# michel-aractingi/soloRL

Hardware: AMD Instinct MI355X
Metric: env-steps/s (whole node) Solo12 walk, 4096 envs/GPU (higher is better)
Workload: dtype f32

## Files before the change

### solorl_amd/csrc/dynamics.hpp

```cpp
#pragma once
#include <utility>

#include "../../include/solorl.h"
#include "../../include/solorl_model_data.h"
#include "spatial.hpp"

namespace solo {

constexpr int MAX_CONTACTS = 8;
constexpr int MAX_LIMITS = 4;
constexpr int LIM_SLOT_ROWS = 2;
constexpr int MAX_ROWS = LIM_SLOT_ROWS + 3 * MAX_CONTACTS;
SD int extra_limits(int nlt) { return nlt > LIM_SLOT_ROWS ? nlt - LIM_SLOT_ROWS : 0; }
SD int contact_cap(int nlt) { return MAX_CONTACTS - extra_limits(nlt); }
constexpr int ROW_CORE = 20;
constexpr int NPRIM = 24;
constexpr double LIMIT_WINDOW = 0.0;
constexpr double DISC_EPS2 = 1e-12;
constexpr double DISC_RIM = 0.1;

#if defined(SOLO_WAVE_TIMING) && !defined(SOLO_HOST_SHIM)
constexpr int SOLO_WT_WAVES = 65536, SOLO_WT_FIELDS = 30;
__device__ unsigned long long solo_wave_times[SOLO_WT_WAVES][SOLO_WT_FIELDS];
__shared__ unsigned long long solo_pt_acc[12];
// ... 1841 lines not shown
    T nz = cw * z + ax * yq - ay * x + az * ww;
    T nq = cw * ww - ax * x - ay * yq - az * z;
    T inv = rsqrt_fast(nx * nx + ny * ny + nz * nz + nq * nq);
    C.ps.qx = nx * inv; C.ps.qy = ny * inv; C.ps.qz = nz * inv; C.ps.qw = nq * inv;
  }
}

template <typename T, int ROBOT, typename LDS> struct TeamCtx {
  using type = CtxLds<T, ROBOT, TeamRows<T, LDS>::off_ctx>;
  static constexpr size_t bytes = TeamRows<T, LDS>::off_ctx + 4 * sizeof(SubCtx<T, ROBOT>);
};

template <typename T, int ROBOT, typename LDS, typename CH>
SNI_SCALAR void duo_helper_rates(CH ch, const PhysParams<T> pp, const LDS lds, int t, bool valid) {
  if (valid) phase_legrates_team<T, ROBOT, LDS, CH>(ch, pp, lds, t);
  WG_SYNC();
}

template <typename T, int ROBOT>
SNI_SCALAR void duo_join_rows() {
  WG_SYNC();
}

template <typename T, int ROBOT, typename LDS, typename CH>
SNI_SCALAR void duo_integrate_joints(CH ch, const PhysParams<T> pp, const LDS lds, int t, bool valid) {
  using RB = Robot<ROBOT>;
  using TRW = TeamRows<T, LDS>;
  constexpr int NJ = RB::NJ, LN = LDS::LANES;
  if (!valid) return;
  SubCtx<T, ROBOT>& C = ch.get();
  const T dt = pp.dt;
  const int mask = C.mask;
  const int nlt = C.nlim_total;
  const T* hdr = lds.hdr();
  const SV<T> w{{hdr[2 * LN], hdr[3 * LN], hdr[4 * LN]}, {hdr[5 * LN], hdr[6 * LN], hdr[7 * LN]}};
  const int tj = t < RB::NQ ? t : 0;
  const int L = tj / NJ, k = tj - L * NJ;
  const T qds = C.qds[tj], yk = lds.y()[(L * 3 + k) * LN], qj = C.ps.q[tj];
  const SV<T> Gk = C.LR[L].G[k];
  const T* lam = TRW::lam(lds.lane);
  const int npos0 = TRW::NPOS0 + extra_limits(nlt);
  T lv[(NPRIM + 15) / 16];
#pragma unroll
  for (int i = 0; i < (NPRIM + 15) / 16; i++) {
    const int p = t + 16 * i;
    const int pp_ = p < NPRIM ? p : 0;
    lv[i] = lam[(npos0 + __builtin_popcount(mask & ((1 << pp_) - 1))) * 4];
    lv[i] = (p < NPRIM && ((mask >> pp_) & 1)) ? lv[i] : T(0);
  }
  const T nvj = clampv(qds + yk - dot(Gk, w), pp.vmax);
#pragma unroll
  for (int i = 0; i < (NPRIM + 15) / 16; i++) { const int p = t + 16 * i; if (p < NPRIM) C.lamp[p] = lv[i]; }
  if (t < RB::NQ) { C.ps.qd[t] = nvj; C.ps.q[t] = qj + dt * nvj; }
}

template <typename T, int ROBOT, typename LDS, typename CH>
SNI_SCALAR void duo_integrate_base(CH ch, const PhysParams<T> pp, const LDS lds, bool lead, bool r0) {
  constexpr int LN = LDS::LANES;
  if (!lead) return;
  SubCtx<T, ROBOT>& C = ch.get();
  const T dt = pp.dt;
  const T* hdr = lds.hdr();
  const SV<T> w{{hdr[2 * LN], hdr[3 * LN], hdr[4 * LN]}, {hdr[5 * LN], hdr[6 * LN], hdr[7 * LN]}};
  const SV<T> ub = C.ub;
  const V3<T> pos = C.ps.pos;
  const T x = C.ps.qx, yq = C.ps.qy, z = C.ps.qz, ww = C.ps.qw;
  const V3<T> nw = mk(clampv(ub.a.x + w.a.x, pp.vmax), clampv(ub.a.y + w.a.y, pp.vmax), clampv(ub.a.z + w.a.z, pp.vmax));
  const V3<T> nv = mk(clampv(ub.l.x + w.l.x, pp.vmax), clampv(ub.l.y + w.l.y, pp.vmax), clampv(ub.l.z + w.l.z, pp.vmax));
  C.ps.w = nw; C.ps.v = nv;
  C.ps.pos = fma3(nv, dt, pos);
  T wn2 = dot(nw, nw), wn = sqrt_fast(wn2), sc, s_, cw;
  sincos_t(T(0.5) * wn * dt, s_, cw);
  if (wn < T(1e-3)) sc = T(0.5) * dt - dt * dt * dt * T(1.0 / 48.0) * wn2; else sc = s_ * rcp_fast(wn);
  T ax = nw.x * sc, ay = nw.y * sc, az = nw.z * sc;
  T nx = cw * x + ax * ww + ay * z - az * yq;
  T ny = cw * yq - ax * z + ay * ww + az * x;
  T nz = cw * z + ax * yq - ay * x + az * ww;
  T nq = cw * ww - ax * x - ay * yq - az * z;
  T inv = rsqrt_fast(nx * nx + ny * ny + nz * nz + nq * nq);
  C.ps.qx = nx * inv; C.ps.qy = ny * inv; C.ps.qz = nz * inv; C.ps.qw = nq * inv;
  if (r0) C.R0 = quat_to_mat(C.ps.qx, C.ps.qy, C.ps.qz, C.ps.qw);
}

template <typename T, int ROBOT, typename LDS>
SD void substep_team_helper(const PhysParams<T> pp, const LDS& lds, int t, bool lead, bool valid, bool r0_next) {
  using CH = typename TeamCtx<T, ROBOT, LDS>::type;
  const CH ch{lds.lane};
  WG_SYNC();
  if (pp.urdf_inertia()) phase_front_team<T, ROBOT, LDS, CH, true, true>(ch, pp, lds, t, valid, lead);
  else phase_front_team<T, ROBOT, LDS, CH, false, true>(ch, pp, lds, t, valid, lead);
  WG_SYNC();
#if defined(SOLO_WAVE_TIMING)
  __builtin_amdgcn_s_waitcnt(0);
  const long long wt_h0_ = clock64();
#endif
  if (valid) team_sum_base<T, ROBOT, CH>(ch, t);
  if (lead) phase_base_lead<T, ROBOT, LDS, CH>(ch, pp, nullptr, 0u, lds);
  else if (!valid && t == 0) {
    lds.hdr()[0] = T(0); lds.hdr()[LDS::LANES] = T(0);
  }
#if defined(SOLO_WAVE_TIMING)
  __builtin_amdgcn_s_waitcnt(0);
  if (threadIdx.x == 64) solo_pt_acc[4] += (unsigned long long)(clock64() - wt_h0_);
#endif
  duo_helper_rates<T, ROBOT, LDS, CH>(ch, pp, lds, t, valid);
  duo_join_rows<T, ROBOT>();
#if defined(SOLO_WAVE_TIMING)
  __builtin_amdgcn_s_waitcnt(0);
  const long long wt_h1_ = clock64();
#endif
  duo_integrate_base<T, ROBOT, LDS, CH>(ch, pp, lds, lead, r0_next);
#if defined(SOLO_WAVE_TIMING)
  __builtin_amdgcn_s_waitcnt(0);
  if (threadIdx.x == 64) solo_pt_acc[11] += (unsigned long long)(clock64() - wt_h1_);
#endif
}

template <typename T, int ROBOT, typename LDS, bool DUO = false>
SD int substep_team(const PhysParams<T> pp, T* lam_prev, unsigned nstride, const LDS& lds, int t, bool lead, bool valid) {
  constexpr int LN = LDS::LANES;
  using TRW = TeamRows<T, LDS>;
  using CH = typename TeamCtx<T, ROBOT, LDS>::type;
  const CH ch{lds.lane};
  SOLO_PT_DECL();
  SOLO_PT_BEGIN();
  if (valid && t < Robot<ROBOT>::NQ) {
    SubCtx<T, ROBOT>& C = ch.get();
    T sn, cs;
    sincos_t(C.ps.q[t], sn, cs);
    C.sn[t] = sn; C.cs[t] = cs;
  }
  SOLO_PT(0);
  const bool ui = pp.urdf_inertia();
  if constexpr (DUO) WG_SYNC();
  else if (ui) phase_front_team<T, ROBOT, LDS, CH, true>(ch, pp, lds, t, valid, lead);
  else phase_front_team<T, ROBOT, LDS, CH, false>(ch, pp, lds, t, valid, lead);
  SOLO_PT(1);
#if SOLO_LEG_QUAD
  if constexpr (DUO) {
    if (ui) phase_leg_rt<T, ROBOT, LDS, CH, true, true>(ch, pp, lam_prev, nstride, lds, t >> 2, t & 3);
    else phase_leg_rt<T, ROBOT, LDS, CH, false, true>(ch, pp, lam_prev, nstride, lds, t >> 2, t & 3);
  } else if (valid) {
    if (ui) phase_leg_rt<T, ROBOT, LDS, CH, true>(ch, pp, lam_prev, nstride, lds, t >> 2, t & 3);
    else phase_leg_rt<T, ROBOT, LDS, CH, false>(ch, pp, lam_prev, nstride, lds, t >> 2, t & 3);
  }
#else
  static_assert(!DUO, "the helper wavefront's barrier B is in the quad leg phase");
  if (valid && t < 4) {
    if (ui) phase_leg_rt<T, ROBOT, LDS, CH, true>(ch, pp, lam_prev, nstride, lds, t, 0);
    else phase_leg_rt<T, ROBOT, LDS, CH, false>(ch, pp, lam_prev, nstride, lds, t, 0);
  }
#endif
  SOLO_PT(2);
  if constexpr (DUO) {
    duo_join_rows<T, ROBOT>();
    SOLO_PT(3);
  } else {
    if (valid) team_sum_base<T, ROBOT, CH>(ch, t);
    SOLO_PT(3);
    if (lead) phase_base_lead<T, ROBOT, LDS, CH>(ch, pp, lam_prev, nstride, lds);
    else if (!valid && t == 0) {
      lds.hdr()[0] = T(0); lds.hdr()[LN] = T(0);
    }
    SOLO_PT(4);
    if (valid) phase_legrates_team<T, ROBOT, LDS, CH>(ch, pp, lds, t);
    SOLO_PT(5);
  }
  phase_finish_team<T, ROBOT, LDS>(pp, lds, t);
  SOLO_PT(6);
  phase_pgs_team<T, ROBOT, LDS>(pp.iterations, pp.warm != T(0), pp.resid_thr >= T(0), pp.pgs_pipe(), pp.cone(), lds, t);
  SOLO_PT(7);
  if constexpr (DUO) {
    duo_join_rows<T, ROBOT>();
    SOLO_PT(10);
    duo_integrate_joints<T, ROBOT, LDS, CH>(ch, pp, lds, t, valid);
  } else phase_integrate_team<T, ROBOT, LDS, CH>(ch, pp, lam_prev, nstride, lds, t, valid, lead);
  SOLO_PT(8);
  return lead ? (ch.get().mask | strip_feet_bits(ch.get().smask)) : 0;
}
#endif

template <typename T, int ROBOT, typename LDS>
SD int substep(SubCtx<T, ROBOT>& C, const PhysParams<T> pp, T* lam_prev, unsigned nstride, const LDS& lds) {
  using CH = CtxPriv<T, ROBOT>;
  const CH ch{&C};
  if (pp.urdf_inertia()) {
    phase_detect<T, ROBOT, CH, true>(ch, pp);
    phase_leg<T, ROBOT, 0, LDS, CH, true>(ch, pp, lam_prev, nstride, lds);
// ... 19 lines not shown
```

### solorl_amd/csrc/solorl_hip.hip

```cpp
#include <hip/hip_runtime.h>

#include <cmath>
#include <cstddef>
#include <cstdio>
#include <cstdlib>
#include <cstring>
#include <utility>
#include <string>
#include <vector>

#include "../../include/solorl.h"
#include "dynamics.hpp"

using namespace solo;

#ifndef SOLO_TU_PART
#define SOLO_TU_PART -1
#endif
extern "C" __attribute__((visibility("hidden"))) int solorl_fail_(int code, const char* msg);

namespace {

#if SOLO_TU_PART == -1 || SOLO_TU_PART == 4
thread_local std::string g_err;
// ... 335 lines not shown
      for (int j = 0; j < NQ; j++) C.tau[j] = tau[j] * sc;
      E.mask = substep<T, ROBOT>(C, pp, sf + SX(L.lam, e, L.NF), 4u, lds);
    }
    E.ps = C.ps;
  }
  if (P.task == SOLORL_TASK_POINTGOAL && mode == MODE_STEP) pointgoal_progress(E, P, P.id0 + (long long)env);
  if (mode == MODE_SETTLE) { store_env(E, sf, si, L, (idx_t)N, e); return; }
  E.timestep += 1;
  const int done = reward_termination_outputs<T, NQ>(E, P, asq, out, env, N);

  if (done) reset_from_snapshot<T, ROBOT>(E, sf, L, (idx_t)N, e, env, snf, sni, M, P);
  write_obs<T, ROBOT>(E, sf, L, (idx_t)N, e, env, P.task, out.obs);
  store_env(E, sf, si, L, (idx_t)N, e);
}

#ifdef SOLO_WAVE_TIMING
#define WT_STAMP(i) do { wts_[i] = clock64(); } while (0)
#else
#define WT_STAMP(i) do {} while (0)
#endif

template <typename T> SD T team_sum16(T x) {
  if constexpr (sizeof(T) == 4) {
    x += __int_as_float(__builtin_amdgcn_mov_dpp(__float_as_int(x), 0xB1, 0xF, 0xF, true));
    x += __int_as_float(__builtin_amdgcn_mov_dpp(__float_as_int(x), 0x4E, 0xF, 0xF, true));
    x += __int_as_float(__builtin_amdgcn_mov_dpp(__float_as_int(x), 0x141, 0xF, 0xF, true));
    x += __int_as_float(__builtin_amdgcn_mov_dpp(__float_as_int(x), 0x140, 0xF, 0xF, true));
  } else {
    x += __shfl_xor(x, 1, 16); x += __shfl_xor(x, 2, 16); x += __shfl_xor(x, 4, 16); x += __shfl_xor(x, 8, 16);
  }
  return x;
}
enum { ER_GOAL = 0, ER_POT = 2, ER_PROG = 3, ER_GOALS = 4, ER_EGOALS = 5, ER_DR = 6, ER_XYPREV = 11, ER_TMY = 13, NER = 14 };
enum { IR_TIMESTEP = 0, IR_MASK = 1, IR_RNG = 2, IR_SNAP = 3, IR_DONE = 4 };
template <typename T, int ROBOT> SD void env_from_lds(Env<T, Robot<ROBOT>::NQ>& E, const SubCtx<T, ROBOT>& C) {
  E.ps = C.ps;
  E.goal[0] = C.erec[ER_GOAL]; E.goal[1] = C.erec[ER_GOAL + 1]; E.pot = C.erec[ER_POT]; E.prog = C.erec[ER_PROG];
  E.goals = C.erec[ER_GOALS]; E.egoals = C.erec[ER_EGOALS];
#pragma unroll
  for (int k = 0; k < 5; k++) E.dr[k] = C.erec[ER_DR + k];
  E.xyprev[0] = C.erec[ER_XYPREV]; E.xyprev[1] = C.erec[ER_XYPREV + 1]; E.tmy = C.erec[ER_TMY];
  E.timestep = C.irec[IR_TIMESTEP]; E.mask = C.irec[IR_MASK]; E.rng = C.irec[IR_RNG];
}
template <typename T, int ROBOT> SD void scalars_to_lds(const Env<T, Robot<ROBOT>::NQ>& E, SubCtx<T, ROBOT>& C) {
  C.erec[ER_GOAL] = E.goal[0]; C.erec[ER_GOAL + 1] = E.goal[1]; C.erec[ER_POT] = E.pot; C.erec[ER_PROG] = E.prog;
  C.erec[ER_GOALS] = E.goals; C.erec[ER_EGOALS] = E.egoals;
#pragma unroll
  for (int k = 0; k < 5; k++) C.erec[ER_DR + k] = E.dr[k];
  C.erec[ER_XYPREV] = E.xyprev[0]; C.erec[ER_XYPREV + 1] = E.xyprev[1]; C.erec[ER_TMY] = E.tmy;
  C.irec[IR_TIMESTEP] = E.timestep; C.irec[IR_MASK] = E.mask; C.irec[IR_RNG] = E.rng;
}

template <typename T, int ROBOT, int HK_>
SD void team_current_state(const SubCtx<T, ROBOT>& C, int task, int D, int t, T (&cs)[HK_]) {
  constexpr int NQ = Robot<ROBOT>::NQ;
  using PS_ = PhysState<T, NQ>;
  static_assert(offsetof(PS_, v) == 7 * sizeof(T) && offsetof(PS_, q) == 13 * sizeof(T) && sizeof(PS_) == (13 + 2 * NQ) * sizeof(T),
                "PhysState is a flat array: pos 0-2, quat 3-6, v 7-9, w 10-12, q, qd");
  const T* psv = reinterpret_cast<const T*>(&C.ps);
  const int mask = C.irec[IR_MASK];
  const T g0 = C.erec[ER_GOAL], g1 = C.erec[ER_GOAL + 1];
  T ang = T(0);
  if (t >= 1 && t <= 3) {
    T r, p, y;
    euler_zyx(C.ps.qx, C.ps.qy, C.ps.qz, C.ps.qw, r, p, y);
    const T a = t == 1 ? r : (t == 2 ? p : y);
    ang = (a - T(2) * floor(a * T(0.5))) * T(0.5);
  }
#pragma unroll
  for (int k = 0; k < HK_; k++) {
    const int d = t + 16 * k;
    const int e = d - (14 + 2 * NQ);
    const int idx = d == 0 ? 2 : (d < 10 + 2 * NQ ? d + 3 : (e >= 0 && e < 2 ? e : 0));
    const T raw = psv[idx];
    const T sc = d < 10 ? T(1) : (d < 10 + NQ ? T(0.1) : (d < 10 + 2 * NQ ? T(0.01) : T(0.5)));
    T v = raw * sc;
    if (d >= 1 && d <= 3) v = ang;
    const int f = d - (10 + 2 * NQ);
    if (f >= 0 && f < 4) v = ((mask >> (13 + 2 * f)) & 1) ? T(1) : T(0);
    if (e == 2) v = g0 * T(0.5);
    if (e == 3) v = g1 * T(0.5);
    if (task != SOLORL_TASK_POINTGOAL && e >= 0) v = T(0);
    cs[k] = d < D ? v : T(0);
  }
}

constexpr float POL_HALF_LOG_2PI = 0.91893853320467274178f;
constexpr unsigned POL_ENV_BYTES = 2496;
static_assert(POL_ENV_BYTES == MAX_ROWS * (ROW_CORE + 4) * sizeof(float), "the policy tail's per-env slice is one env's fp32 row storage (RowLds)");
static_assert((224 + 128) * sizeof(float) <= POL_ENV_BYTES, "the last activation block (h2: 128 floats at float offset 224) must end inside the slice");
SD float pol_tanh(float x) { const float e = __expf(2.0f * x); return 1.0f - 2.0f * __builtin_amdgcn_rcpf(1.0f + e); }
typedef float nfloat4 __attribute__((ext_vector_type(4)));
typedef __attribute__((address_space(1))) const nfloat4 gfloat4;
SD float pol_dot4(nfloat4 w, nfloat4 x, float acc) { return fmaf(w.x, x.x, fmaf(w.y, x.y, fmaf(w.z, x.z, fmaf(w.w, x.w, acc)))); }
#define POL_PIN4(x) asm volatile("" : "+v"(x))
template <int KB> struct PolBatch { nfloat4 c[KB], a[KB]; };
template <int KB>
SD void pol_load(PolBatch<KB>& B, const float* wc_, const float* wa_, int K4, int k0, int lane) {
  gfloat4* wc = (gfloat4*)(wc_ + (size_t)lane * 4 * K4);
  gfloat4* wa = (gfloat4*)(wa_ + (size_t)lane * 4 * K4);
#pragma unroll
  for (int kk = 0; kk < KB; kk++) {
    const int k = k0 + kk < K4 ? k0 + kk : K4 - 1;
    B.c[kk] = wc[k]; B.a[kk] = wa[k];
  }
  asm volatile("" ::: "memory");
}
template <int KB>
SD void pol_fma(PolBatch<KB>& B, int K4, int k0, unsigned xoff, unsigned xoff_a, float (&c)[4], float (&a)[4]) {
  asm volatile("" ::: "memory");
#pragma unroll
  for (int kk = 0; kk < KB; kk++) { POL_PIN4(B.c[kk]); POL_PIN4(B.a[kk]); }
#pragma unroll
  for (int kk = 0; kk < KB; kk++)
    if (k0 + kk < K4) {
#pragma unroll
      for (int e = 0; e < 4; e++) {
        const nfloat4 xc = reinterpret_cast<const nfloat4*>(solo_smem + e * POL_ENV_BYTES + xoff)[k0 + kk];
        const nfloat4 xa = xoff_a == xoff ? xc : reinterpret_cast<const nfloat4*>(solo_smem + e * POL_ENV_BYTES + xoff_a)[k0 + kk];
        c[e] = pol_dot4(B.c[kk], xc, c[e]); a[e] = pol_dot4(B.a[kk], xa, a[e]);
      }
    }
}
SD void pol_act_store(const float (&c)[4], const float (&a)[4], unsigned yoff, int lane) {
#pragma unroll
  for (int e = 0; e < 4; e++) {
    float* y = reinterpret_cast<float*>(solo_smem + e * POL_ENV_BYTES + yoff);
    y[lane] = pol_tanh(c[e]); y[64 + lane] = pol_tanh(a[e]);
  }
}

template <int A>
SD void policy_tail_team(const PolicyTail& P, int O, int col, int t, idx_t env, bool valid) {
  float* const buf = reinterpret_cast<float*>(solo_smem + (unsigned)col * POL_ENV_BYTES);
  float* const h2 = buf + 224;
  const int lane = threadIdx.x & 63, O4 = O >> 2;
  static_assert(A < 15, "the critic head sits on lane 15");
  const bool head = t < A || t == 15;
  constexpr unsigned H1 = 96u * 4u, H2 = 224u * 4u;
  float c[4], a[4];
  PolBatch<11> w1a, w1b;
  PolBatch<8> w2a, w2b;
  nfloat4 whb[16];
  pol_load(w1a, P.cw0, P.aw0, O4, 0, lane);
  pol_load(w1b, P.cw0, P.aw0, O4, 11, lane);
#pragma unroll
  for (int e = 0; e < 4; e++) { c[e] = P.cb0[lane]; a[e] = P.ab0[lane]; }
  pol_fma(w1a, O4, 0, 0u, 0u, c, a);
  pol_load(w2a, P.cw1, P.aw1, 16, 0, lane);
  pol_fma(w1b, O4, 11, 0u, 0u, c, a);
  pol_act_store(c, a, H1, lane);
  pol_load(w2b, P.cw1, P.aw1, 16, 8, lane);
#pragma unroll
  for (int e = 0; e < 4; e++) { c[e] = P.cb1[lane]; a[e] = P.ab1[lane]; }
  TEAM_SYNC();
  pol_fma(w2a, 16, 0, H1, H1 + 256u, c, a);
  {
    gfloat4* wh = (gfloat4*)(t == 15 ? P.cw2 : P.mw + (size_t)(head ? t : 0) * 64);
#pragma unroll
    for (int k = 0; k < 16; k++) whb[k] = wh[k];
    asm volatile("" ::: "memory");
  }
  pol_fma(w2b, 16, 8, H1, H1 + 256u, c, a);
  pol_act_store(c, a, H2, lane);
  TEAM_SYNC();
  float out = 0.f;
  {
    asm volatile("" ::: "memory");
#pragma unroll
    for (int k = 0; k < 16; k++) POL_PIN4(whb[k]);
    const nfloat4* x = reinterpret_cast<const nfloat4*>(t == 15 ? h2 : h2 + 64);
    float o0 = t == 15 ? P.cb2[0] : P.mb[head ? t : 0], o1 = 0.f;
#pragma unroll
    for (int k = 0; k < 16; k += 2) { o0 = pol_dot4(whb[k], x[k], o0); o1 = pol_dot4(whb[k + 1], x[k + 1], o1); }
    out = head ? o0 + o1 : 0.f;
  }
  float lp = 0.f, act = out;
  if (t < A) {
    const float ls = P.logstd[t];
    const float nz = P.noise ? P.noise[(size_t)env * A + t] : 0.f;
    act = out + __expf(ls) * nz;
    lp = -0.5f * nz * nz - ls - POL_HALF_LOG_2PI;
  }
  lp = team_sum16(lp);
  if (valid) {
    if (t < A) P.action[(size_t)env * A + t] = act;
    if (t == 15) P.value[env] = out;
    if (t == 0) P.logp[env] = lp;
  }
}

template <typename T, int ROBOT, bool DUO = false>
SD void step_team(T* __restrict__ sf, int* __restrict__ si, const T* __restrict__ snf, const int* __restrict__ sni, int M,
                  const Layout& L, int N, const EnvParams& P, const PhysParams<T>& pp, const float* __restrict__ actions,
                  const Outputs& out, int mode) {
  using RB = Robot<ROBOT>;
  constexpr int NQ = RB::NQ, NPS = 13 + 2 * NQ;
  using LDS = RowLds<T, 4>;
  using CH = typename TeamCtx<T, ROBOT, LDS>::type;
  static_assert(sizeof(PhysState<T, NQ>) == NPS * sizeof(T), "PhysState is the HBM field order pos, quat, v, w, q, qd");
#ifdef SOLO_WAVE_TIMING
  long long wts_[11];
  for (int i_ = 0; i_ < 11; i_++) wts_[i_] = 0;
  const long long wr0_ = wall_clock64();
  if (threadIdx.x < 12) solo::solo_pt_acc[threadIdx.x] = 0;
  __syncthreads();
  wts_[0] = clock64();
#endif
  const unsigned wlane = DUO ? (threadIdx.x & 63u) : threadIdx.x;
  const int t = wlane & 15, col = wlane >> 4;
  const unsigned blk = (blockIdx.x & 7u) * (gridDim.x >> 3) + (blockIdx.x >> 3);
  idx_t e = (idx_t)blk * 4 + col;
  const bool valid = e < (idx_t)N;
  if (!valid) e = (idx_t)N - 1;
  const bool lead = valid && t == 0;
  LDS lds; lds.lanes = 4; lds.lane = col;
  if (P.lds_poison_on) {
    using TC = TeamCtx<T, ROBOT, LDS>;
    unsigned* w = reinterpret_cast<unsigned*>(solo_smem);
    for (unsigned k = wlane; k < TC::bytes / 4; k += 64) w[k] = P.lds_poison;
    __syncthreads();
  }
  const CH ch{col};
  SubCtx<T, ROBOT>& C = ch.get();
  T* const psv = reinterpret_cast<T*>(&C.ps);
  if constexpr (DUO) {
    if (blk * 4u >= (unsigned)N) return;
    if (__builtin_amdgcn_readfirstlane(threadIdx.x >> 6)) {
#pragma unroll 1
      for (int ss = 0; ss < P.frame_skip; ss++)
        substep_team_helper<T, ROBOT>(pp, lds, t, lead, valid, ss + 1 < P.frame_skip);
      duo_join_rows<T, ROBOT>();
      return;
    }
    if (!valid && t == 0) { C.mask = 0; C.nc = 0; C.nlim_total = 0; C.lsel = 0; C.smask = 0; }
  }
  idx_t env = 0;
  T a_t = T(0);
  if (valid) {
    env = P.linear_ids ? e : (idx_t)si[SX(I_ENVID, e, NI)];
    for (int f = t; f < NPS; f += 16) psv[f] = sf[SX(L.pos + f, e, L.NF)];
    if (t < NER) C.erec[t] = sf[SX(L.goal + t, e, L.NF)];
    if (t < 3) C.irec[t] = si[SX(t, e, NI)];
    for (int p = t; p < NPRIM; p += 16) C.lamp[p] = sf[SX(L.lam + p, e, L.NF)];
    if (t < NQ && mode == MODE_STEP) a_t = (T)actions[env * NQ + t];
  }
  static_assert(I_TIMESTEP == IR_TIMESTEP && I_MASK == IR_MASK && I_RNG == IR_RNG, "counter order");
  TEAM_SYNC();
  WT_STAMP(1);
  if (valid && t < NQ) {
    const T c = a_t < T(-1) ? T(-1) : (a_t > T(1) ? T(1) : a_t);
    T tq;
    if (P.control == SOLORL_CONTROL_TORQUE) tq = c * T(P.max_torque);
    else tq = clampv(T(P.kp) * (c * pp.qlim - C.ps.q[t]) - T(P.kd) * C.ps.qd[t], T(P.max_torque));
    C.tau_base[t] = mode == MODE_STEP ? tq : T(0);
    if (out.tau && mode == MODE_STEP) out.tau[env * NQ + t] = (float)tq;
  }
  const T asq = team_sum16(a_t * a_t);
  WT_STAMP(2);
  constexpr int HK = (DMAX + 15) / 16;
  T hk0[HK], hk1[HK];
#pragma unroll
  for (int k = 0; k < HK; k++) { hk0[k] = T(0); hk1[k] = T(0); }
  T csk[HK];
  if (L.H > 0) team_current_state<T, ROBOT, HK>(C, P.task, L.D, t, csk);
  TEAM_SYNC();
  if (lead) {
    C.erec[ER_XYPREV] = C.ps.pos.x; C.erec[ER_XYPREV + 1] = C.ps.pos.y;
    C.tmy = C.erec[ER_TMY];
    if constexpr (DUO) C.R0 = quat_to_mat(C.ps.qx, C.ps.qy, C.ps.qz, C.ps.qw);
  }
  if (valid && L.H > 0) {
#pragma unroll
    for (int k = 0; k < HK; k++) {
      const int d = t + 16 * k;
      if (d < L.D) {
        const T c = csk[k];
        for (int lv = L.H - 1; lv >= 2; lv--)
          sf[SX(L.hist + lv * HSTRIDE + d, e, L.NF)] = sf[SX(L.hist + (lv - 1) * HSTRIDE + d, e, L.NF)];
        if (L.H >= 2) { hk1[k] = sf[SX(L.hist + d, e, L.NF)]; sf[SX(L.hist + HSTRIDE + d, e, L.NF)] = hk1[k]; }
        sf[SX(L.hist + d, e, L.NF)] = c;
        hk0[k] = c;
      } else if (d < ((L.D + 3) & ~3)) {
        sf[SX(L.hist + d, e, L.NF)] = T(0);
        for (int lv = 1; lv < L.H; lv++) sf[SX(L.hist + lv * HSTRIDE + d, e, L.NF)] = T(0);
      }
    }
  }
  WT_STAMP(3);
#pragma unroll 1
  for (int ss = 0; ss < P.frame_skip; ss++) {
    const T sc = (ss == 0 || P.hold_torque) ? T(1) : T(0);
    if (valid && t < NQ) C.tau[t] = C.tau_base[t] * sc;
    const int m = substep_team<T, ROBOT, LDS, DUO>(pp, sf + SX(L.lam, e, L.NF), 4u, lds, t, lead, valid);
    if (lead) C.irec[IR_MASK] = m;
  }
  if constexpr (DUO) {
    duo_join_rows<T, ROBOT>();
  }
  WT_STAMP(4);
  if (valid) for (int p = t; p < NPRIM; p += 16) sf[SX(L.lam + p, e, L.NF)] = C.lamp[p];
  WT_STAMP(5);
  if (lead) {
    Env<T, NQ> E;
    env_from_lds<T, ROBOT>(E, C);
    int done = 0;
    if (P.task == SOLORL_TASK_POINTGOAL && mode == MODE_STEP) pointgoal_progress(E, P, P.id0 + (long long)env);
    if (mode == MODE_STEP) {
      E.timestep += 1;
      done = reward_termination_outputs<T, NQ>(E, P, asq, out, env, N);
      if (done) C.irec[IR_SNAP] = reset_draws(E, P, P.id0 + (long long)env);
    }
    scalars_to_lds<T, ROBOT>(E, C);
    C.irec[IR_DONE] = done;
  }
  WT_STAMP(6);
  TEAM_SYNC();
  const int done = valid ? C.irec[IR_DONE] : 0;
  if (done) {
    const idx_t k = (idx_t)C.irec[IR_SNAP], MM = (idx_t)M;
    for (int f = t; f < L.NF; f += 16) {
      const T v = snf[SX(f, k, L.NF)];
      const bool scalar = f >= L.goal && f < L.goal + NER;
      if (!scalar) sf[SX(f, e, L.NF)] = v;
      if (f < NPS) psv[f] = v;
      else if (scalar && f != L.goal && f != L.goal + 1) C.erec[f - L.goal] = v;
    }
    if (t == 1) C.irec[IR_MASK] = sni[SX(I_MASK, k, NI)];
#pragma unroll
    for (int kk = 0; kk < HK; kk++) {
      const int d = t + 16 * kk;
      if (d < L.D) {
        if (L.H >= 1) hk0[kk] = snf[SX(L.hist + d, k, L.NF)];
        if (L.H >= 2) hk1[kk] = snf[SX(L.hist + HSTRIDE + d, k, L.NF)];
      }
    }
    TEAM_SYNC();
    const T g0 = C.erec[ER_GOAL], g1 = C.erec[ER_GOAL + 1];
    if (P.task == SOLORL_TASK_POINTGOAL) {
#pragma unroll
      for (int kk = 0; kk < HK; kk++) {
        const int d = t + 16 * kk;
        if (d == L.D - 2 || d == L.D - 1) {
          const T gv = (d == L.D - 2 ? g0 : g1) * T(0.5);
          if (L.H >= 1) { hk0[kk] = gv; sf[SX(L.hist + d, e, L.NF)] = gv; }
          if (L.H >= 2) { hk1[kk] = gv; sf[SX(L.hist + HSTRIDE + d, e, L.NF)] = gv; }
          for (int lv = 2; lv < L.H; lv++) sf[SX(L.hist + lv * HSTRIDE + d, e, L.NF)] = gv;
        }
      }
    }
    if (t == 0) {
      C.irec[IR_TIMESTEP] = 0;
      C.erec[ER_GOALS] = T(0); C.erec[ER_EGOALS] = T(0);
#pragma unroll
      for (int q = 0; q < 5; q++) C.erec[ER_DR + q] = T(0);
      if (P.task == SOLORL_TASK_POINTGOAL) {
        const T dx = C.ps.pos.x - g0, dy = C.ps.pos.y - g1, px = C.erec[ER_XYPREV] - g0, py = C.erec[ER_XYPREV + 1] - g1;
        const T pot = sqrt(dx * dx + dy * dy);
        C.erec[ER_POT] = pot; C.erec[ER_PROG] = -(pot - sqrt(px * px + py * py));
      }
    }
  }
  WT_STAMP(7);
  const bool want_obs = mode == MODE_STEP;
  TEAM_SYNC();
  T cso[HK];
  if (want_obs) team_current_state<T, ROBOT, HK>(C, P.task, L.D, t, cso);
  WT_STAMP(8);
  bool with_policy = false;
  if constexpr (sizeof(T) == 4) with_policy = want_obs && out.pol.value != nullptr;
  if (valid) {
    if (want_obs) {
      float* o = out.obs + env * (idx_t)(L.D * (1 + L.H));
      float* ol = reinterpret_cast<float*>(solo_smem + (unsigned)col * POL_ENV_BYTES);
#pragma unroll
      for (int k = 0; k < HK; k++) {
        const int d = t + 16 * k;
        if (d < L.D) {
          const T c = cso[k];
          o[d] = (float)c;
          if (L.H >= 1) o[L.D + d] = (float)(c - hk0[k]);
          if (L.H >= 2) o[2 * L.D + d] = (float)(c - hk1[k]);
          for (int lv = 2; lv < L.H; lv++) {
            T hv;
            if (done) {
              hv = snf[SX(L.hist + lv * HSTRIDE + d, (idx_t)C.irec[IR_SNAP], L.NF)];
              if (P.task == SOLORL_TASK_POINTGOAL && d >= L.D - 2) hv = C.erec[ER_GOAL + (d - (L.D - 2))] * T(0.5);
            } else hv = sf[SX(L.hist + lv * HSTRIDE + d, e, L.NF)];
            o[(lv + 1) * L.D + d] = (float)(c - hv);
          }
          if (with_policy) {
            ol[d] = (float)c;
            if (L.H >= 1) ol[L.D + d] = (float)(c - hk0[k]);
          }
        }
      }
    }
    for (int f = t; f < ((NPS + 3) & ~3); f += 16) sf[SX(L.pos + f, e, L.NF)] = f < NPS ? psv[f] : T(0);
    sf[SX(L.goal + t, e, L.NF)] = t < NER ? C.erec[t] : T(0);
    if (t < 3) si[SX(t, e, NI)] = C.irec[t];
  }
  if constexpr (sizeof(T) == 4) {
    if (with_policy) {
      TEAM_SYNC();
      policy_tail_team<NQ>(out.pol, L.D * (1 + L.H), col, t, env, valid);
    }
  }
  WT_STAMP(9);
#ifdef SOLO_WAVE_TIMING
  __builtin_amdgcn_s_waitcnt(0);
  if (threadIdx.x == 0 && blockIdx.x < solo::SOLO_WT_WAVES) {
    wts_[10] = clock64();
    unsigned long long* w_ = solo::solo_wave_times[blockIdx.x];
    w_[0] = (unsigned long long)(wts_[3] - wts_[0]); w_[1] = (unsigned long long)(wts_[4] - wts_[3]); w_[2] = (unsigned long long)(wts_[10] - wts_[4]);
    w_[3] = (unsigned long long)(wall_clock64() - wr0_);
    for (int i_ = 0; i_ < 10; i_++) w_[6 + i_] = (unsigned long long)(wts_[i_ + 1] > wts_[i_] && wts_[i_] ? wts_[i_ + 1] - wts_[i_] : 0);
    for (int i_ = 0; i_ < 10; i_++) w_[16 + i_] = solo::solo_pt_acc[i_];
    for (int i_ = 10; i_ < 12; i_++) w_[18 + i_] = solo::solo_pt_acc[i_];
  }
#endif
}

template <typename T, int ROBOT>
__global__ void __launch_bounds__(64)
step_kernel(T* __restrict__ sf, int* __restrict__ si, const T* __restrict__ snf, const int* __restrict__ sni, int M,
            Layout L, int N, EnvParams P, PhysParams<T> pp, const float* __restrict__ actions, Outputs out, int mode) {
  step_body<T, ROBOT>(sf, si, snf, sni, M, L, N, P, pp, actions, out, mode);
}

#ifndef SOLO_WAVES_PER_SIMD
#define SOLO_WAVES_PER_SIMD 2
#endif
template <typename T, int ROBOT>
__global__ void __launch_bounds__(64, sizeof(T) == 8 ? 1 : SOLO_WAVES_PER_SIMD)
step_kernel_team(T* __restrict__ sf, int* __restrict__ si, const T* __restrict__ snf, const int* __restrict__ sni, int M,
                 Layout L, int N, EnvParams P, PhysParams<T> pp, const float* __restrict__ actions, Outputs out, int mode) {
  step_team<T, ROBOT>(sf, si, snf, sni, M, L, N, P, pp, actions, out, mode);
}

template <typename T, int ROBOT>
__global__ void __launch_bounds__(128, SOLO_WAVES_PER_SIMD)
duo_kernel_team(T* __restrict__ sf, int* __restrict__ si, const T* __restrict__ snf, const int* __restrict__ sni, int M,
                Layout L, int N, EnvParams P, PhysParams<T> pp, const float* __restrict__ actions, Outputs out, int mode) {
  static_assert(sizeof(T) == 4, "the helper wavefront is an fp32 kernel");
  step_team<T, ROBOT, true>(sf, si, snf, sni, M, L, N, P, pp, actions, out, mode);
}

template <typename T> struct RolloutArgs {
  T* sf; int* si; const T* snf; const int* sni; int M;
  Layout L; int N; EnvParams P; PhysParams<T> pp;
  const float* actions; Outputs out;
  int mode;
  int K, pol_last;
};
template <typename T> SD T* row_adv(T* p, size_t n) { return p ? p + n : p; }
template <typename T, int ROBOT>
__global__ void __launch_bounds__(64, sizeof(T) == 8 ? 1 : SOLO_WAVES_PER_SIMD)
rollout_kernel_team(const RolloutArgs<T> args) {
  using RA = RolloutArgs<T>;
  typedef const __attribute__((address_space(4))) char* kptr;
  constexpr size_t A = Robot<ROBOT>::NQ;
  const int K = args.K;
#pragma unroll 1
  for (int k = 0; k < K; k++) {
    kptr ap = (kptr)__builtin_amdgcn_kernarg_segment_ptr();
    asm volatile("" : "+s"(ap));
    const RA& a = *(const RA*)ap;
    const size_t r = (size_t)k * (size_t)a.N, O = (size_t)(a.L.D * (1 + a.L.H));
    Outputs o = a.out;
    o.obs += r * O; o.rew += r; o.done += r;
    o.timeout = row_adv(o.timeout, r); o.success = row_adv(o.success, r); o.nan_reset = row_adv(o.nan_reset, r);
    o.ep_len = row_adv(o.ep_len, r); o.ep_rew = row_adv(o.ep_rew, r); o.goals = row_adv(o.goals, r);
    o.dr0 = row_adv(o.dr0, r); o.dr1 = row_adv(o.dr1, r); o.dr2 = row_adv(o.dr2, r); o.dr3 = row_adv(o.dr3, r); o.dr4 = row_adv(o.dr4, r);
    o.tau = row_adv(o.tau, r * A);
    if (o.pol.value) {
      if (k + 1 < K || a.pol_last) {
        const size_t r1 = r + (size_t)a.N;
        o.pol.value += r1; o.pol.logp += r1; o.pol.action += r1 * A; o.pol.noise = row_adv(o.pol.noise, r1 * A);
      } else o.pol.value = nullptr;
    }
    step_team<T, ROBOT>(a.sf, a.si, a.snf, a.sni, a.M, a.L, a.N, a.P, a.pp, a.actions + r * A, o, a.mode);
    TEAM_SYNC();
  }
}

template <typename T, int ROBOT, bool MASKED>
__global__ void reset_kernel(T* sf, int* si, const T* snf, const int* sni, int M, Layout L, int N, EnvParams P, float* obs,
                             const unsigned char* mask) {
  const idx_t e = (idx_t)blockIdx.x * blockDim.x + threadIdx.x;
  if (e >= (idx_t)N) return;
  if constexpr (MASKED) { if (!mask[si[SX(I_ENVID, e, NI)]]) return; }
  Env<T, Robot<ROBOT>::NQ> E;
  load_env(E, sf, si, L, (idx_t)N, e);
  const idx_t env = (idx_t)si[SX(I_ENVID, e, NI)];
  reset_from_snapshot<T, ROBOT>(E, sf, L, (idx_t)N, e, env, snf, sni, M, P);
  if (obs) write_obs<T, ROBOT>(E, sf, L, (idx_t)N, e, env, P.task, obs);
  store_env(E, sf, si, L, (idx_t)N, e);
  si[SX(I_NEEDRESET, e, NI)] = 0;
}

template <typename T, int ROBOT>
__global__ void obs_kernel(const T* sf, const int* si, Layout L, int N, int task, float* obs) {
  const idx_t e = (idx_t)blockIdx.x * blockDim.x + threadIdx.x;
  if (e >= (idx_t)N) return;
  Env<T, Robot<ROBOT>::NQ> E;
  load_env(E, sf, si, L, (idx_t)N, e);
  write_obs<T, ROBOT>(E, sf, L, (idx_t)N, e, (idx_t)si[SX(I_ENVID, e, NI)], task, obs);
}

template <typename T>
__global__ void init_pose_kernel(T* sf, int* si, Layout L, int N, T tmy) {
  const idx_t e = (idx_t)blockIdx.x * blockDim.x + threadIdx.x;
  if (e >= (idx_t)N) return;
  for (int f = 0; f < L.NF; f++) sf[SX(f, e, L.NF)] = T(0);
  sf[SX(L.pos + 2, e, L.NF)] = T(0.35);
  sf[SX(L.quat + 3, e, L.NF)] = T(1);
  sf[SX(L.tmy, e, L.NF)] = tmy;
  for (int k = 0; k < NI; k++) si[SX(k, e, NI)] = 0;
  si[SX(I_NEEDRESET, e, NI)] = 1;
  si[SX(I_ENVID, e, NI)] = (int)e;
}

template <typename T>
__global__ void copy_env_kernel(const T* sf, const int* si, int N, int src, T* df, int* di, int M, int dst, int NF) {
  const int f = blockIdx.x * blockDim.x + threadIdx.x;
  if (f < NF) df[SX(f, (idx_t)dst, NF)] = sf[SX(f, (idx_t)src, NF)];
  if (f < NI) di[SX(f, (idx_t)dst, NI)] = si[SX(f, (idx_t)src, NI)];
// ... 226 lines not shown
  bool f64 = false, reset_called = false;
  size_t tsize = 4;
  Layout L;
  void* sf = nullptr; int* si = nullptr; void* snf = nullptr; int* sni = nullptr;
  void* sf2 = nullptr; int* si2 = nullptr; int* perm = nullptr;
  bool sort = true;
  uint64_t seed = 0; int64_t id0 = 0;
  double goal_radius = 2.0;
  double* dyn = nullptr;
  std::vector<unsigned> stab_host;
  unsigned* stab = nullptr;
  bool spread = true;
  bool team = false;
  int lds_poison_on = 0; unsigned lds_poison = 0;
  int simds = 1024;
  int pipe_override = -1;
  int helper_override = -1;
};

namespace {

EnvParams make_env_params(const solorl_env* h) {
  EnvParams P;
  const solorl_config& c = h->cfg;
  P.task = c.task; P.control = c.control; P.frame_skip = c.frame_skip; P.episode_length = c.episode_length;
  P.hold_torque = c.hold_torque; P.disable_termination = c.disable_termination;
  P.settle_min = c.settle_min; P.nsettle = c.settle_max - c.settle_min + 1;
  P.seed_lo = (unsigned)h->seed; P.seed_hi = (unsigned)(h->seed >> 32); P.id0 = h->id0;
  P.kp = c.kp; P.kd = c.kd; P.max_torque = c.max_torque; P.reward_dt = c.reward_dt; P.dyn = h->dyn;
  P.lds_poison_on = h->lds_poison_on; P.lds_poison = h->lds_poison;
  P.use_treadmill = c.use_treadmill; P.tm_offset = (float)c.treadmill_offset;
  P.linear_ids = h->sort ? 0 : 1;
  return P;
}

inline int check_lds_base(const void* kernel) {
  hipFuncAttributes a;
  HIP_TRY(hipFuncGetAttributes(&a, kernel));
  if (a.sharedSizeBytes != (size_t)SOLO_LDS_BASE)
    return fail(SOLORL_ERR_HIP, "step kernel's static LDS size differs from SOLO_LDS_BASE: the phase functions' dynamic-LDS base constant does not hold "
                                "(a -DSOLO_WAVE_TIMING build runs team mode only)");
  return 0;
}

inline int team_grid(int N) { return (((N + 3) / 4) + 7) & ~7; }
inline bool team_pipe(const solorl_env* h, int N) { return h->pipe_override >= 0 ? h->pipe_override != 0 : team_grid(N) <= h->simds; }
inline bool helper_wave_allowed(const solorl_env* h) { return h->team && !h->f64 && !h->sort && team_grid(h->N) <= h->simds; }
inline bool helper_wave_rule(const solorl_env* h) { return h->helper_override != 0 && helper_wave_allowed(h); }
inline bool step_n_one_launch(const solorl_env* h) { return h->team && !h->sort; }

template <typename T, int ROBOT>
PhysParams<T> team_launch_shape(const solorl_env* h, int N, dim3& grid, size_t& smem) {
  grid = dim3(team_grid(N));
  using TeamLds = RowLds<T, 4>;
  smem = TeamCtx<T, ROBOT, TeamLds>::bytes;
  static_assert(sizeof(T) == 8 || TeamCtx<T, ROBOT, TeamLds>::bytes <= 20480, "team-mode LDS must allow 8 workgroups per CU (two wavefronts per SIMD)");
  PhysParams<T> pp = make_phys<T>(h->cfg);
  pp.mode = (pp.mode & ~PhysParams<T>::M_PIPE) | (team_pipe(h, N) ? PhysParams<T>::M_PIPE : 0);
  return pp;
}

template <typename T, int ROBOT>
int prepare_kernels(const solorl_env* h) {
  if (int rc = check_lds_base(h->team ? reinterpret_cast<const void*>(step_kernel_team<T, ROBOT>) : reinterpret_cast<const void*>(step_kernel<T, ROBOT>))) return rc;
  if constexpr (sizeof(T) == 4)
    if (helper_wave_rule(h))
      if (int rc = check_lds_base(reinterpret_cast<const void*>(duo_kernel_team<T, ROBOT>))) return rc;
  if (step_n_one_launch(h))
    if (int rc = check_lds_base(reinterpret_cast<const void*>(rollout_kernel_team<T, ROBOT>))) return rc;
  if (!h->team)
    HIP_TRY(hipFuncSetAttribute(reinterpret_cast<const void*>(step_kernel<T, ROBOT>), hipFuncAttributeMaxDynamicSharedMemorySize,
                                (int)RowLds<T>::bytes(sizeof(T) == 8 ? 32 : 64)));
  return 0;
}

template <typename T, int ROBOT>
int launch_step(solorl_env* h, T* sf, int* si, int N, const float* actions, const Outputs& out, int mode, hipStream_t st) {
  if (h->team) {
    dim3 grid;
    size_t team_smem = 0;
    const PhysParams<T> pp = team_launch_shape<T, ROBOT>(h, N, grid, team_smem);
    if constexpr (sizeof(T) == 4) {
      if (helper_wave_rule(h)) {
        hipLaunchKernelGGL((duo_kernel_team<T, ROBOT>), grid, dim3(128), team_smem, st, sf, si, (const T*)h->snf, (const int*)h->sni, h->M, h->L, N,
                           make_env_params(h), pp, actions, out, mode);
        HIP_TRY(hipGetLastError());
        return 0;
      }
    }
    hipLaunchKernelGGL((step_kernel_team<T, ROBOT>), grid, dim3(64), team_smem, st, sf, si, (const T*)h->snf, (const int*)h->sni, h->M, h->L, N,
                       make_env_params(h), pp, actions, out, mode);
    HIP_TRY(hipGetLastError());
    return 0;
  }
  const int EPB = RowLds<T>::LANES;
  size_t smem = RowLds<T>::bytes(EPB);
  if (h->spread && (N + EPB - 1) / EPB <= 256) smem = RowLds<T>::bytes(sizeof(T) == 8 ? 32 : 64);
  dim3 grid((N + EPB - 1) / EPB), block(EPB);
  hipLaunchKernelGGL((step_kernel<T, ROBOT>), grid, block, smem, st, sf, si, (const T*)h->snf, (const int*)h->sni, h->M, h->L, N,
                     make_env_params(h), make_phys<T>(h->cfg), actions, out, mode);
  HIP_TRY(hipGetLastError());
  return 0;
}

template <typename T, int ROBOT>
int launch_rollout(solorl_env* h, T* sf, int* si, int N, const float* actions, const Outputs& out, int K, int pol_last, hipStream_t st) {
  dim3 grid, block(64);
  RolloutArgs<T> a;
  size_t smem = 0;
  a.pp = team_launch_shape<T, ROBOT>(h, N, grid, smem);
  a.sf = sf; a.si = si; a.snf = (const T*)h->snf; a.sni = (const int*)h->sni; a.M = h->M; a.L = h->L; a.N = N; a.P = make_env_params(h);
  a.actions = actions; a.out = out; a.mode = MODE_STEP; a.K = K; a.pol_last = pol_last;
  hipLaunchKernelGGL((rollout_kernel_team<T, ROBOT>), grid, block, smem, st, a);
  HIP_TRY(hipGetLastError());
  return 0;
}

}

#define SOLO_LAUNCH_ARGS solorl_env* h, void* sf, int* si, int N, const float* actions, const void* out, int mode, void* st
#define SOLO_ROLLOUT_ARGS solorl_env* h, void* sf, int* si, int N, const float* actions, const void* out, int K, int pol_last, void* st
#define SOLO_DECLARE_PART(K_) \
  extern "C" __attribute__((visibility("hidden"))) int solorl_prepare_part##K_(const solorl_env* h); \
  extern "C" __attribute__((visibility("hidden"))) int solorl_launch_part##K_(SOLO_LAUNCH_ARGS); \
  extern "C" __attribute__((visibility("hidden"))) int solorl_rollout_part##K_(SOLO_ROLLOUT_ARGS);
SOLO_DECLARE_PART(0) SOLO_DECLARE_PART(1) SOLO_DECLARE_PART(2) SOLO_DECLARE_PART(3)
#define SOLO_DEFINE_PART(K_, T_, R_) \
  extern "C" int solorl_prepare_part##K_(const solorl_env* h) { return prepare_kernels<T_, R_>(h); } \
  extern "C" int solorl_launch_part##K_(SOLO_LAUNCH_ARGS) { \
    return launch_step<T_, R_>(h, (T_*)sf, si, N, actions, *(const Outputs*)out, mode, (hipStream_t)st); } \
  extern "C" int solorl_rollout_part##K_(SOLO_ROLLOUT_ARGS) { \
    return launch_rollout<T_, R_>(h, (T_*)sf, si, N, actions, *(const Outputs*)out, K, pol_last, (hipStream_t)st); }
#if SOLO_TU_PART == -1 || SOLO_TU_PART == 0
SOLO_DEFINE_PART(0, float, 0)
#endif
#if SOLO_TU_PART == -1 || SOLO_TU_PART == 1
SOLO_DEFINE_PART(1, float, 1)
#endif
#if SOLO_TU_PART == -1 || SOLO_TU_PART == 2
SOLO_DEFINE_PART(2, double, 0)
#endif
#if SOLO_TU_PART == -1 || SOLO_TU_PART == 3
SOLO_DEFINE_PART(3, double, 1)
#endif

#if SOLO_TU_PART == -1 || SOLO_TU_PART == 4
namespace {

template <typename F> auto with_type(const solorl_env* h, F&& f) { return h->f64 ? f(double{}) : f(float{}); }
template <typename F> auto with_instantiation(const solorl_env* h, F&& f) {
  return with_type(h, [&](auto t) {
    return h->cfg.robot == SOLORL_ROBOT_SOLO12 ? f(t, std::integral_constant<int, 1>{}) : f(t, std::integral_constant<int, 0>{});
  });
}

int part_index(const solorl_env* h) { return 2 * (h->f64 ? 1 : 0) + (h->cfg.robot == SOLORL_ROBOT_SOLO12 ? 1 : 0); }
constexpr decltype(&solorl_launch_part0) PART_LAUNCH[4] = {solorl_launch_part0, solorl_launch_part1, solorl_launch_part2, solorl_launch_part3};
constexpr decltype(&solorl_rollout_part0) PART_ROLLOUT[4] = {solorl_rollout_part0, solorl_rollout_part1, solorl_rollout_part2, solorl_rollout_part3};
constexpr decltype(&solorl_prepare_part0) PART_PREPARE[4] = {solorl_prepare_part0, solorl_prepare_part1, solorl_prepare_part2, solorl_prepare_part3};

int dispatch_step(solorl_env* h, void* sf, int* si, int N, const float* actions, const Outputs& out, int mode, hipStream_t st) {
  return PART_LAUNCH[part_index(h)](h, sf, si, N, actions, &out, mode, st);
}

int dispatch_rollout(solorl_env* h, const float* actions, const Outputs& out, int K, int pol_last, hipStream_t st) {
  return PART_ROLLOUT[part_index(h)](h, h->sf, h->si, h->N, actions, &out, K, pol_last, st);
}
// ... 514 lines not shown
```

Baseline: 28.88 million.

## Move history state capture to helper wave and prefetch duo kernargs

In the two-wave duo kernel, the helper wave now computes the current observation state during the first substep's idle slot and stages it in extra LDS. The main wave later reads it to shift the observation history, instead of computing it on its own critical path. The launch also touches all kernarg cache lines up front to warm them, and uses a fixed LDS size that still allows four workgroups per CU. The cost is extra LDS plus a dependence on the staged data staying valid until the history update runs.

```diff
diff --git a/solorl_amd/csrc/dynamics.hpp b/solorl_amd/csrc/dynamics.hpp
--- a/solorl_amd/csrc/dynamics.hpp
+++ b/solorl_amd/csrc/dynamics.hpp
@@ -1947,8 +1947,8 @@
   if (r0) C.R0 = quat_to_mat(C.ps.qx, C.ps.qy, C.ps.qz, C.ps.qw);
 }
 
-template <typename T, int ROBOT, typename LDS>
-SD void substep_team_helper(const PhysParams<T> pp, const LDS& lds, int t, bool lead, bool valid, bool r0_next) {
+template <typename T, int ROBOT, typename LDS, typename MID>
+SD void substep_team_helper(const PhysParams<T> pp, const LDS& lds, int t, bool lead, bool valid, bool r0_next, const MID& mid) {
   using CH = typename TeamCtx<T, ROBOT, LDS>::type;
   const CH ch{lds.lane};
   WG_SYNC();
@@ -1969,6 +1969,15 @@
   if (threadIdx.x == 64) solo_pt_acc[4] += (unsigned long long)(clock64() - wt_h0_);
 #endif
   duo_helper_rates<T, ROBOT, LDS, CH>(ch, pp, lds, t, valid);
+#if defined(SOLO_WAVE_TIMING)
+  __builtin_amdgcn_s_waitcnt(0);
+  const long long wt_h2_ = clock64();
+#endif
+  mid();
+#if defined(SOLO_WAVE_TIMING)
+  __builtin_amdgcn_s_waitcnt(0);
+  if (threadIdx.x == 64) solo_pt_acc[5] += (unsigned long long)(clock64() - wt_h2_);
+#endif
   duo_join_rows<T, ROBOT>();
 #if defined(SOLO_WAVE_TIMING)
   __builtin_amdgcn_s_waitcnt(0);
diff --git a/solorl_amd/csrc/solorl_hip.hip b/solorl_amd/csrc/solorl_hip.hip
--- a/solorl_amd/csrc/solorl_hip.hip
+++ b/solorl_amd/csrc/solorl_hip.hip
@@ -441,6 +441,28 @@
     if (e == 3) v = g1 * T(0.5);
     if (task != SOLORL_TASK_POINTGOAL && e >= 0) v = T(0);
     cs[k] = d < D ? v : T(0);
+  }
+}
+
+template <typename T, int ROBOT> struct DuoStage {
+  static constexpr size_t off = (TeamCtx<T, ROBOT, RowLds<T, 4>>::bytes + 15) & ~(size_t)15;
+  static constexpr size_t bytes = off + (size_t)4 * DMAX * sizeof(T);
+  SD static T* row(int col) { return reinterpret_cast<T*>(solo_smem + off) + col * DMAX; }
+};
+
+template <typename T, int ROBOT>
+SNI_SCALAR void duo_history_state(int task, int D, int col, int t) {
+  using CH = typename TeamCtx<T, ROBOT, RowLds<T, 4>>::type;
+  constexpr int HK = (DMAX + 15) / 16;
+  t &= 15; col &= 3;
+  const CH ch{col};
+  T cs[HK];
+  team_current_state<T, ROBOT, HK>(ch.get(), task, D, t, cs);
+  T* st = DuoStage<T, ROBOT>::row(col);
+#pragma unroll
+  for (int k = 0; k < HK; k++) {
+    const int d = t + 16 * k;
+    if (d < D) st[d] = cs[k];
   }
 }
 
@@ -577,7 +599,8 @@
   if (P.lds_poison_on) {
     using TC = TeamCtx<T, ROBOT, LDS>;
     unsigned* w = reinterpret_cast<unsigned*>(solo_smem);
-    for (unsigned k = wlane; k < TC::bytes / 4; k += 64) w[k] = P.lds_poison;
+    constexpr size_t words = (DUO ? DuoStage<T, ROBOT>::bytes : TC::bytes) / 4;
+    for (unsigned k = wlane; k < words; k += 64) w[k] = P.lds_poison;
     __syncthreads();
   }
   const CH ch{col};
@@ -588,7 +611,10 @@
     if (__builtin_amdgcn_readfirstlane(threadIdx.x >> 6)) {
 #pragma unroll 1
       for (int ss = 0; ss < P.frame_skip; ss++)
-        substep_team_helper<T, ROBOT>(pp, lds, t, lead, valid, ss + 1 < P.frame_skip);
+        substep_team_helper<T, ROBOT>(pp, lds, t, lead, valid, ss + 1 < P.frame_skip,
+                                      [on = ss == 0 && valid && L.H > 0, task = P.task, D = L.D, col, t]() {
+          if (on) duo_history_state<T, ROBOT>(task, D, col, t);
+        });
       duo_join_rows<T, ROBOT>();
       return;
     }
@@ -622,14 +648,14 @@
 #pragma unroll
   for (int k = 0; k < HK; k++) { hk0[k] = T(0); hk1[k] = T(0); }
   T csk[HK];
-  if (L.H > 0) team_current_state<T, ROBOT, HK>(C, P.task, L.D, t, csk);
+  if constexpr (!DUO) { if (L.H > 0) team_current_state<T, ROBOT, HK>(C, P.task, L.D, t, csk); }
   TEAM_SYNC();
   if (lead) {
     C.erec[ER_XYPREV] = C.ps.pos.x; C.erec[ER_XYPREV + 1] = C.ps.pos.y;
     C.tmy = C.erec[ER_TMY];
     if constexpr (DUO) C.R0 = quat_to_mat(C.ps.qx, C.ps.qy, C.ps.qz, C.ps.qw);
   }
-  if (valid && L.H > 0) {
+  if (!DUO && valid && L.H > 0) {
 #pragma unroll
     for (int k = 0; k < HK; k++) {
       const int d = t + 16 * k;
@@ -717,6 +743,26 @@
         const T dx = C.ps.pos.x - g0, dy = C.ps.pos.y - g1, px = C.erec[ER_XYPREV] - g0, py = C.erec[ER_XYPREV + 1] - g1;
         const T pot = sqrt(dx * dx + dy * dy);
         C.erec[ER_POT] = pot; C.erec[ER_PROG] = -(pot - sqrt(px * px + py * py));
+      }
+    }
+  }
+  if constexpr (DUO) {
+    if (valid && !done && L.H > 0) {
+      const T* st = DuoStage<T, ROBOT>::row(col);
+#pragma unroll
+      for (int k = 0; k < HK; k++) {
+        const int d = t + 16 * k;
+        if (d < L.D) {
+          const T c = st[d];
+          for (int lv = L.H - 1; lv >= 2; lv--)
+            sf[SX(L.hist + lv * HSTRIDE + d, e, L.NF)] = sf[SX(L.hist + (lv - 1) * HSTRIDE + d, e, L.NF)];
+          if (L.H >= 2) { hk1[k] = sf[SX(L.hist + d, e, L.NF)]; sf[SX(L.hist + HSTRIDE + d, e, L.NF)] = hk1[k]; }
+          sf[SX(L.hist + d, e, L.NF)] = c;
+          hk0[k] = c;
+        } else if (d < ((L.D + 3) & ~3)) {
+          sf[SX(L.hist + d, e, L.NF)] = T(0);
+          for (int lv = 1; lv < L.H; lv++) sf[SX(L.hist + lv * HSTRIDE + d, e, L.NF)] = T(0);
+        }
       }
     }
   }
@@ -797,11 +843,25 @@
   step_team<T, ROBOT>(sf, si, snf, sni, M, L, N, P, pp, actions, out, mode);
 }
 
+template <typename T> struct DuoKernargs {
+  T* sf; int* si; const T* snf; const int* sni; int M;
+  Layout L; int N; EnvParams P; PhysParams<T> pp;
+  const float* actions; Outputs out; int mode;
+};
+template <typename T, size_t... I>
+SD void duo_touch_kernargs(std::index_sequence<I...>) {
+  typedef const __attribute__((address_space(4))) unsigned* kptr;
+  kptr ap = (kptr)__builtin_amdgcn_kernarg_segment_ptr();
+  const unsigned any = (ap[I * 16] | ... | ap[(offsetof(DuoKernargs<T>, mode)) / 4]);
+  asm volatile("" :: "s"(any));
+}
+
 template <typename T, int ROBOT>
 __global__ void __launch_bounds__(128, SOLO_WAVES_PER_SIMD)
 duo_kernel_team(T* __restrict__ sf, int* __restrict__ si, const T* __restrict__ snf, const int* __restrict__ sni, int M,
                 Layout L, int N, EnvParams P, PhysParams<T> pp, const float* __restrict__ actions, Outputs out, int mode) {
   static_assert(sizeof(T) == 4, "the helper wavefront is an fp32 kernel");
+  duo_touch_kernargs<T>(std::make_index_sequence<(sizeof(DuoKernargs<T>) + 63) / 64>());
   step_team<T, ROBOT, true>(sf, si, snf, sni, M, L, N, P, pp, actions, out, mode);
 }
 
@@ -1194,7 +1254,9 @@
     const PhysParams<T> pp = team_launch_shape<T, ROBOT>(h, N, grid, team_smem);
     if constexpr (sizeof(T) == 4) {
       if (helper_wave_rule(h)) {
-        hipLaunchKernelGGL((duo_kernel_team<T, ROBOT>), grid, dim3(128), team_smem, st, sf, si, (const T*)h->snf, (const int*)h->sni, h->M, h->L, N,
+        static_assert(DuoStage<T, ROBOT>::bytes <= 40960, "the duo launch's LDS must allow 4 workgroups per CU (one per SIMD)");
+        constexpr size_t duo_smem = DuoStage<T, ROBOT>::bytes;
+        hipLaunchKernelGGL((duo_kernel_team<T, ROBOT>), grid, dim3(128), duo_smem, st, sf, si, (const T*)h->snf, (const int*)h->sni, h->M, h->L, N,
                            make_env_params(h), pp, actions, out, mode);
         HIP_TRY(hipGetLastError());
         return 0;
```

After: 29.12 million (median of 6 runs). No clear change (+0.8%).
